# ZenGo-X/multi-party-ecdsa

Hardware: AMD Instinct MI355X
Metric: GG20 signatures/sec (t=1, n=3; all parties of each session on the node's GPUs) + Paillier-2048 modexp/s per GPU (higher is better)
Workload: dtype u32 limbs (radix 2^29) / u64 accumulators

## Files before the change

multi_party_ecdsa_amd/csrc/mpe_internal.h:

```cpp
#pragma once
#include <hip/hip_runtime.h>
#include <stdint.h>
#include <new>
#include <utility>
#include <string>
#include <vector>

#include "../../include/mpecdsa_hip.h"
#include "mpe_kernels_heavy.h"
#include "mpe_sched.h"

struct mpe_ctx {
  int device = 0;
  int cus = 256;
  int fb_window_bits = 13;
  int window_bits = 0;
  bool ec_lane_groups = true;
  bool adaptive_lanes = true;
  bool use_pown = true;
  bool use_pair = true;
  bool use_multiexp = true;
  bool use_crt = true;
  bool use_fixed_base = true;
  bool use_sliding = true;
  int wide_div = 4;
  int device_share = 1;
  int xwide_div = 16;
  bool merge_xn = true;
  int use_prio = 1;
  int ladder_prio = 1;
  int use_crt_n = 1;
  int no_pdl_ahead = 0;
  int no_r1_dlog_first = 0;
  int no_r1_inversion_ahead = 0;
  int merge_r1_quarters = 1;
  bool merge_r1 = true;
  size_t fb_budget_bytes = 0;
  int modexp_waves_per_cu = 8;
  int fb_split = 0;
  int gg20_trace = 0;
  int sampler_max_attempts = 128;
  int no_primaries = 0;
  int no_elect = 0;
  int grid_mode = 2;
  void* tables[6] = {nullptr, nullptr, nullptr, nullptr, nullptr, nullptr};
  size_t tables_bytes[6] = {0, 0, 0, 0, 0, 0};
  hipStream_t aux[3] = {nullptr, nullptr, nullptr};
  hipEvent_t ev_fork[2] = {nullptr, nullptr}, ev_join[3] = {nullptr, nullptr, nullptr};
  hipEvent_t ev_ahead = nullptr;
  hipEvent_t ev_mid = nullptr;
  bool aux_ready = false;
  bool allow_par = true;
  int par_items = 32768;
  void* ws = nullptr;
  size_t ws_bytes = 0, ws_off = 0;
  int ws_hold = 0;
  size_t ws_top = 0;
  void* sess_buf = nullptr;
  size_t sess_bytes = 0;
  bool sess_in_use = false;
  void* slab_buf = nullptr;
  size_t slab_bytes = 0;
  mpe_launch_info last = {};
  mpe_encoding enc = {};
  bool prof_on = false;
  struct ProfEvt { hipEvent_t a, b; int kind, bits, exp_words, batch, exp2_words; int wave_trips; };
  std::vector<ProfEvt> prof;
  uint32_t* prof_ctr = nullptr;
  int prof_ctr_cap = 0;
};

struct mpe_modset {
// ... 98 lines not shown
```

multi_party_ecdsa_amd/csrc/mpe_lib.hip:

```cpp
#include <string.h>
#include <initializer_list>
#include <mutex>
#include "mpe_internal.h"
#include "mpe_ec.h"

using namespace mpe;

thread_local std::string g_last_error;
void mpe_set_error(const char* what, hipError_t e) { g_last_error = std::string(what) + ": " + hipGetErrorString(e); }
void mpe_set_error_msg(const char* what) { g_last_error = what; }

namespace mpe {

int ws_reserve(mpe_ctx* ctx, size_t bytes, hipStream_t st) {
  if (ctx->ws_hold) {
    if (ctx->ws_off + bytes + ctx->ws_top > ctx->ws_bytes) { mpe_set_error_msg("workspace: the shared reservation is too small"); return MPE_E_NOMEM; }
    return MPE_OK;
  }
  ctx->ws_off = 0;
  if (bytes + ctx->ws_top <= ctx->ws_bytes) return MPE_OK;
  if (ctx->ws_top) { mpe_set_error_msg("workspace: cannot grow while a caller keeps arrays at its top"); return MPE_E_NOMEM; }
  if (ctx->ws) { (void)hipStreamSynchronize(st); (void)hipFree(ctx->ws); ctx->ws = nullptr; ctx->ws_bytes = 0; }
  const size_t want = bytes + (bytes >> 2) + (1u << 20);
  hipError_t e = hipMalloc(&ctx->ws, want);
// ... 235 lines not shown
extern "C" {

const char* mpe_version(void) { return "mpecdsa-hip 0.6.0 (gfx950)"; }
const char* mpe_last_error(void) { return g_last_error.c_str(); }

void mpe_encoding_default(mpe_encoding* e) {
  if (!e) return;
  memset(e, 0, sizeof *e);
  e->ck_salt = 0x4B5A656Eu;
  for (int i = 0; i < 4; ++i) e->ord_dlog[i] = e->ord_cdlog[i] = (uint8_t)i;
  for (int i = 0; i < 8; ++i) e->ord_pedersen[i] = e->ord_heg[i] = e->ord_ecddh[i] = (uint8_t)i;
}
static bool is_perm(const uint8_t* o, int n) {
  unsigned seen = 0;
  for (int i = 0; i < n; ++i) { if (o[i] >= n || (seen >> o[i]) & 1u) return false; seen |= 1u << o[i]; }
  return true;
}
int mpe_ctx_set_encoding(mpe_ctx* ctx, const mpe_encoding* e) {
  if (!ctx || !e) return MPE_E_ARG;
  if (e->chain_point > 1 || e->zero_bytes > 1 || e->ck_mask_order > 1 || e->reserved != 0 || !is_perm(e->ord_dlog, 3) ||
      !is_perm(e->ord_pedersen, 5) || !is_perm(e->ord_heg, 7) || !is_perm(e->ord_ecddh, 6) || !is_perm(e->ord_cdlog, 4)) {
    mpe_set_error_msg("mpe_ctx_set_encoding: a flag is not 0/1 or an order is not a permutation");
    return MPE_E_ARG;
  }
  ctx->enc = *e;
  return MPE_OK;
}
int mpe_ctx_set_device_share(mpe_ctx* ctx, int contexts) {
  if (!ctx || contexts < 1 || contexts > 64) return MPE_E_ARG;
  ctx->device_share = contexts;
  return MPE_OK;
}
int mpe_ctx_get_encoding(const mpe_ctx* ctx, mpe_encoding* out) {
  if (!ctx || !out) return MPE_E_ARG;
  *out = ctx->enc;
  return MPE_OK;
}

namespace mpe {
struct CtxOption {
  const char* key;
  long lo, hi;
  void (*set)(mpe_ctx*, long);
  long (*get)(const mpe_ctx*);
};
#define MPE_OPT_BOOL_OFF(name, field) {name, 0, 1, [](mpe_ctx* c, long v) { c->field = !v; }, [](const mpe_ctx* c) -> long { return c->field ? 0 : 1; }}
#define MPE_OPT_INT(name, lo, hi, field) {name, lo, hi, [](mpe_ctx* c, long v) { c->field = (decltype(c->field))v; }, [](const mpe_ctx* c) -> long { return (long)c->field; }}
static const CtxOption kCtxOptions[] = {
    MPE_OPT_BOOL_OFF("no_fixed_base", use_fixed_base),
    MPE_OPT_BOOL_OFF("no_crt", use_crt),
    MPE_OPT_BOOL_OFF("no_multiexp", use_multiexp),
    MPE_OPT_BOOL_OFF("no_pair", use_pair),
    MPE_OPT_BOOL_OFF("no_pown", use_pown),
    MPE_OPT_BOOL_OFF("no_sliding", use_sliding),
    MPE_OPT_BOOL_OFF("no_par", allow_par),
    MPE_OPT_BOOL_OFF("no_wide", adaptive_lanes),
    MPE_OPT_BOOL_OFF("no_ec_lane_groups", ec_lane_groups),
    MPE_OPT_BOOL_OFF("no_merge_xn", merge_xn),
    MPE_OPT_BOOL_OFF("no_merge_r1", merge_r1),
    MPE_OPT_INT("fb_window_bits", 4, 16, fb_window_bits),
    MPE_OPT_INT("window_bits", 0, 6, window_bits),
    MPE_OPT_INT("wide_div", 1, 64, wide_div),
    MPE_OPT_INT("merge_r1_quarters", 0, 64, merge_r1_quarters),
    MPE_OPT_INT("no_r1_inversion_ahead", 0, 1, no_r1_inversion_ahead),
    MPE_OPT_BOOL_OFF("no_prio", use_prio),
    MPE_OPT_INT("no_pdl_ahead", 0, 1, no_pdl_ahead),
    MPE_OPT_BOOL_OFF("no_crt_n", use_crt_n),
    MPE_OPT_INT("no_r1_dlog_first", 0, 1, no_r1_dlog_first),
    MPE_OPT_INT("xwide_div", 0, 1 << 20, xwide_div),
    MPE_OPT_INT("waves_per_cu", 1, 8, modexp_waves_per_cu),
    MPE_OPT_INT("grid_mode", 0, 2, grid_mode),
    MPE_OPT_INT("fb_split", 0, 64, fb_split),
    MPE_OPT_INT("gg20_trace", 0, 1, gg20_trace),
    MPE_OPT_INT("sampler_max_attempts", 1, 1 << 20, sampler_max_attempts),
    MPE_OPT_INT("no_primaries", 0, 1, no_primaries),
    MPE_OPT_INT("no_elect", 0, 1, no_elect),
    {"fb_budget_mb", 0, 1 << 20, [](mpe_ctx* c, long v) { c->fb_budget_bytes = (size_t)v << 20; }, [](const mpe_ctx* c) -> long { return (long)(c->fb_budget_bytes >> 20); }},
};
#undef MPE_OPT_BOOL_OFF
#undef MPE_OPT_INT
extern "C++" void ctx_copy_options(mpe_ctx* dst, const mpe_ctx* src) {
  for (const CtxOption& o : kCtxOptions) o.set(dst, o.get(src));
}
}

int mpe_ctx_set_option(mpe_ctx* ctx, const char* key, const char* value) {
  if (!ctx || !key || !value) return MPE_E_ARG;
  if (!strcmp(key, "grid")) {
    const int m = !strcmp(value, "equal") ? 0 : (!strcmp(value, "full") ? 1 : (!strcmp(value, "hybrid") ? 2 : -1));
    if (m < 0) { mpe_set_error_msg("mpe_ctx_set_option: grid = equal | full | hybrid"); return MPE_E_ARG; }
    ctx->grid_mode = m;
    return MPE_OK;
  }
  if (!strcmp(key, "no_adaptive_lanes")) {
    const bool off = atoi(value) != 0;
    ctx->adaptive_lanes = !off; ctx->ec_lane_groups = !off;
    return MPE_OK;
  }
  for (const mpe::CtxOption& o : mpe::kCtxOptions) {
    if (strcmp(key, o.key)) continue;
    char* end = nullptr;
    const long v = strtol(value, &end, 10);
    if (end == value || *end || v < o.lo || v > o.hi) {
      mpe_set_error_msg((std::string("mpe_ctx_set_option: ") + key + " takes an integer in [" + std::to_string(o.lo) + ", " + std::to_string(o.hi) + "]").c_str());
      return MPE_E_ARG;
    }
// ... 205 lines not shown
```

multi_party_ecdsa_amd/csrc/mpe_pairexp.h:

```cpp
#pragma once
#include <type_traits>
#include "mpe_internal.h"
#include "mpe_small.h"

namespace mpe {

template <class C>
struct PairLds {
  static constexpr int B0 = 0;
  static constexpr int B1 = C::K;
  static constexpr int M = 2 * C::K;
  static constexpr int KC = 3 * C::K;
  static constexpr int pick_stride() {
    constexpr int per_half = (C::GROUPS >= 2) ? C::GROUPS / 2 : 1;
    for (int s = 4 * C::K + 2;; s += 2) {
      bool ok = true;
      for (int a = 0; a < per_half && ok; ++a)
        for (int b = a + 1; b < per_half; ++b)
          if (((a * s) & 31) == ((b * s) & 31)) { ok = false; break; }
      if (ok) return s;
    }
  }
  static constexpr int STRIDE = pick_stride();
  static constexpr int WORDS = STRIDE * C::GROUPS;
// ... 66 lines not shown
      const uint32_t bj = bp[r];
      c[r] += (uint64_t)a[0] * bj;
      const uint32_t m = bcast0_masked<C::TPI>((uint32_t)c[r] * n0inv, maskv);
      if (STORE_M) mp[r] = m;
#pragma unroll
      for (int i = 1; i < L; ++i) c[(r + i) % L] += (uint64_t)a[i] * bj;
#pragma unroll
      for (int i = 0; i < L; ++i) c[(r + i) % L] += (uint64_t)m * n[i];
      c[(r + 1) % L] += c[r] >> W;
      c[r] = (uint64_t)(pull_next((uint32_t)c[r]) & maskv);
    };
    static_for<0, C::STEPS % L>(step);
    if (jj == C::STEPS / L) break;
    static_for<C::STEPS % L, L>(step);
  }
  cios_finish<C>(res, c, ln);
}

template <class C>
__device__ __forceinline__ void cios2(uint32_t (&res)[C::L], uint64_t (&c)[C::L], const uint32_t (&a0)[C::L],
                                      const uint32_t (&a1)[C::L], const uint32_t* __restrict__ bl0,
                                      const uint32_t* __restrict__ bl1, const uint32_t (&n)[C::L], uint32_t n0inv,
                                      const Lane& ln) {
  constexpr int L = C::L, W = C::W;
  uint32_t maskv = C::MASK;
  asm volatile("" : "+v"(maskv));
#pragma unroll 1
  for (int jj = 0;; ++jj) {
    const uint32_t* bp0 = bl0 + jj * L;
    const uint32_t* bp1 = bl1 + jj * L;
    auto step = [&](auto rc) {
      constexpr int r = decltype(rc)::value;
      const uint32_t b0j = bp0[r], b1j = bp1[r];
      c[r] += (uint64_t)a0[0] * b1j;
      c[r] += (uint64_t)a1[0] * b0j;
      const uint32_t m = bcast0_masked<C::TPI>((uint32_t)c[r] * n0inv, maskv);
#pragma unroll
      for (int i = 1; i < L; ++i) {
        c[(r + i) % L] += (uint64_t)a0[i] * b1j;
        c[(r + i) % L] += (uint64_t)a1[i] * b0j;
      }
#pragma unroll
      for (int i = 0; i < L; ++i) c[(r + i) % L] += (uint64_t)m * n[i];
      c[(r + 1) % L] += c[r] >> W;
      c[r] = (uint64_t)(pull_next((uint32_t)c[r]) & maskv);
    };
    static_for<0, C::STEPS % L>(step);
    if (jj == C::STEPS / L) break;
    static_for<C::STEPS % L, L>(step);
  }
  cios_finish<C>(res, c, ln);
}

template <class C>
__device__ __forceinline__ void pairmul(uint32_t (&r0)[C::L], uint32_t (&r1)[C::L], const uint32_t (&a0)[C::L],
                                        const uint32_t (&a1)[C::L], uint32_t* gl, const uint32_t (&n)[C::L],
                                        uint32_t n0inv, bool sq, bool half, const Lane& ln) {
  using PL = PairLds<C>;
  constexpr int L = C::L;
  uint64_t c[L];
#pragma unroll
  for (int i = 0; i < L; ++i) c[i] = 0;
  cios1<C, true>(r0, c, a0, gl + PL::B0, gl + PL::M, n, n0inv, ln);
  wave_lds_sync();
  if (half) {
#pragma unroll
    for (int i = 0; i < L; ++i) r1[i] = 0;
    return;
  }
#pragma unroll
  for (int i = 0; i < L; ++i) {
    uint32_t mi = gl[PL::M + ln.t * L + i];
    if (C::STEPS == C::K - 1) {
      if (i == L - 1) mi = (ln.t == C::TPI - 1) ? 0u : mi;
    } else if (C::STEPS < C::K) {
      mi = (ln.t * L + i < C::STEPS) ? mi : 0u;
    }
    c[i] = (uint64_t)(gl[PL::KC + ln.t * L + i] - mi);
  }
  wave_lds_sync();
#pragma unroll
  for (int i = 0; i < L; ++i) gl[PL::M + ln.t * L + i] = r0[i];
  if (sq) {
    cios1<C, false>(r1, c, a1, gl + PL::B1, gl + PL::M, n, n0inv, ln);
  } else {
    cios2<C>(r1, c, a0, a1, gl + PL::B0, gl + PL::B1, n, n0inv, ln);
  }
  wave_lds_sync();
#pragma unroll
  for (int i = 0; i < L; ++i) r0[i] = gl[PL::M + ln.t * L + i];
}

template <class C>
__device__ __forceinline__ void copy_pair_to_lds(uint32_t* gl, const uint32_t* __restrict__ src, const Lane& ln, int off1 = C::K) {
  using PL = PairLds<C>;
#pragma unroll
  for (int i = 0; i < C::L; ++i) {
    gl[PL::B0 + ln.t + C::TPI * i] = src[ln.t + C::TPI * i];
    gl[PL::B1 + ln.t + C::TPI * i] = src[off1 + ln.t + C::TPI * i];
  }
}
template <class C>
__device__ __forceinline__ void copy_row_to_lds(uint32_t* gl, const uint32_t* __restrict__ row, const Lane& ln) {
  using PL = PairLds<C>;
  static_assert(PL::B0 == 0 && PL::B1 == C::K && (2 * C::K) % 4 == 0 && PL::STRIDE % 2 == 0, "B0 | B1 must be one 8-byte aligned run");
  constexpr int CHUNKS = 2 * C::K / 4;
  const uint4* __restrict__ r4 = reinterpret_cast<const uint4*>(row);
  uint2* l2 = reinterpret_cast<uint2*>(gl + PL::B0);
#pragma unroll
  for (int i = 0; i < (CHUNKS + C::TPI - 1) / C::TPI; ++i) {
    const int ch = ln.t + C::TPI * i;
    if ((i + 1) * C::TPI <= CHUNKS || ch < CHUNKS) {
      const uint4 v = r4[ch];
      l2[2 * ch] = make_uint2(v.x, v.y);
      l2[2 * ch + 1] = make_uint2(v.z, v.w);
    }
  }
}

template <class C>
__global__ void __launch_bounds__(64) pairset_setup_kernel(int count, const uint32_t* __restrict__ moduli,
                                                           uint32_t* __restrict__ n_limbs, uint32_t* __restrict__ n0inv_out,
                                                           uint32_t* __restrict__ one, uint32_t* __restrict__ r2,
                                                           uint32_t* __restrict__ tp, uint32_t* __restrict__ kc) {
  __shared__ uint32_t lds[C::LDS_WORDS];
  constexpr int KS = pair_kstore(C::BITS);
  const Lane ln = make_lane<C>();
  uint32_t* gl = lds + ln.g * C::STRIDE;
  const int slot = blockIdx.x * C::GROUPS + ln.g;
  const bool active = slot < count;
  const int idx = active ? slot : count - 1;
  stage_words<C>(gl, moduli + (size_t)idx * C::K32, ln);
  wave_lds_sync();
  uint32_t n[C::L];
  limbs_from_words<C>(n, gl, ln);
  const uint32_t w0 = gl[0];
  uint32_t inv = w0;
#pragma unroll
  for (int i = 0; i < 5; ++i) inv *= 2u - w0 * inv;
  const uint32_t n0inv = (0u - inv) & C::MASK;
  wave_lds_sync();

  int64_t x0[C::L], x1[C::L];
#pragma unroll
  for (int i = 0; i < C::L; ++i) { x0[i] = (ln.t == 0 && i == 0) ? 1 : 0; x1[i] = 0; }
  auto store_pair = [&](uint32_t* dst) {
    if (!active) return;
#pragma unroll
    for (int i = 0; i < C::L; ++i) {
      dst[(size_t)idx * 2 * KS + ln.t * C::L + i] = (uint32_t)x0[i];
      dst[(size_t)idx * 2 * KS + KS + ln.t * C::L + i] = (uint32_t)x1[i];
    }
  };
  constexpr int WK = C::W * C::STEPS;
#pragma unroll 1
  for (int d = 1; d <= 2 * WK; ++d) {
#pragma unroll
    for (int i = 0; i < C::L; ++i) x0[i] *= 2;
    full_normalize<C>(x0, ln);
    const bool cy = cmp_ge<C>(x0, n, ln);
    if (cy) {
#pragma unroll
      for (int i = 0; i < C::L; ++i) x0[i] -= (int64_t)n[i];
      full_normalize<C>(x0, ln);
    }
#pragma unroll
    for (int i = 0; i < C::L; ++i) x1[i] *= 2;
    if (cy && ln.t == 0) x1[0] += 1;
    full_normalize<C>(x1, ln);
    if (cmp_ge<C>(x1, n, ln)) {
#pragma unroll
// ... 59 lines not shown
  __syncthreads();
  for (int k = threadIdx.x; k < nkeys; k += blockDim.x)
    if (sh[k]) atomicAdd(&cnt[k], sh[k]);
}
static __global__ void __launch_bounds__(64) key_scan_kernel(int nkeys, const int32_t* __restrict__ cnt, int32_t* __restrict__ cursor) {
  __shared__ int32_t part[64];
  const int per = (nkeys + 63) / 64, lo = threadIdx.x * per, hi = lo + per < nkeys ? lo + per : nkeys;
  int32_t s = 0;
  for (int k = lo; k < hi; ++k) s += cnt[k];
  part[threadIdx.x] = s;
  __syncthreads();
  int32_t base = 0;
  for (int t = 0; t < (int)threadIdx.x; ++t) base += part[t];
  for (int k = lo; k < hi; ++k) { cursor[k] = base; base += cnt[k]; }
}
static __global__ void __launch_bounds__(256) key_scatter_kernel(int batch, Rows sel, int nkeys, int32_t* __restrict__ cursor, int32_t* __restrict__ perm) {
  extern __shared__ int32_t sh[];
  for (int k = threadIdx.x; k < 2 * nkeys; k += blockDim.x) sh[k] = 0;
  __syncthreads();
  const int i = blockIdx.x * blockDim.x + threadIdx.x;
  const int mi = i < batch ? sel_index(sel, i) : -1;
  const int local = mi >= 0 ? atomicAdd(&sh[mi], 1) : 0;
  __syncthreads();
  for (int k = threadIdx.x; k < nkeys; k += blockDim.x)
    if (sh[k]) sh[nkeys + k] = atomicAdd(&cursor[k], sh[k]);
  __syncthreads();
  if (mi >= 0) perm[sh[nkeys + mi] + local] = i;
}

static __global__ void pair_slide_audit_kernel(int batch, int groups, Rows exps, int exp_words, int wb, int exp2_words,
                                               const int32_t* __restrict__ perm, uint32_t* __restrict__ ctr) {
  const int u = blockIdx.x * blockDim.x + threadIdx.x;
  if (u * groups >= batch) return;
  const uint32_t* first = nullptr;
  bool same = true;
  for (int g = 0; g < groups; ++g) {
    const int inst = u * groups + g;
    const int pos = inst < batch ? inst : batch - 1;
    const uint32_t* ex = row_of(exps, perm ? perm[pos] : pos);
    if (g == 0) first = ex; else same = same && ex == first;
  }
  if (!same) return;
  uint32_t val = 0;
  const int lo = slide_window((UniformWords)(uintptr_t)first, exp_words, exp_words * 32 - 1, wb, val);
  if (lo < 0 || (exp2_words && lo < 32 * exp2_words)) return;
  atomicAdd(ctr, 1u);
}

#ifdef MPE_WAVE_TRACE
static __device__ unsigned long long* g_wave_trace;
static __device__ unsigned g_wave_trace_cap, g_wave_trace_n;
#endif

template <class C, bool SLIDE>
__global__ void __launch_bounds__(64) __attribute__((amdgpu_waves_per_eu(2, 2))) pair_modexp_kernel(int batch, PairsetView ps, Rows mod_sel, Rows base, Rows exps,
                                                         int exp_words, int wb, Rows base2, Rows exps2, int exp2_words,
                                                         int half, uint32_t* __restrict__ out, uint32_t* __restrict__ tables,
                                                         const int32_t* __restrict__ perm, int slide, SchedArgs sched) {
  using PL = PairLds<C>;
  __shared__ __attribute__((aligned(16))) uint32_t lds[PL::WORDS];
  const Lane ln = make_lane<C>();
  uint32_t* gl = lds + ln.g * PL::STRIDE;
  constexpr int K2 = 2 * C::K;
  const int slot = blockIdx.x * C::GROUPS + ln.g;
  const int nslots = gridDim.x * C::GROUPS;
  const bool dual = base2.p != nullptr;
  const int TE = 1 << wb;
  uint32_t* tab = tables + (size_t)slot * (TE + (dual ? 16 : 0)) * K2;
  uint32_t* tab2 = tab + (size_t)TE * K2;
  const int nwin = (exp_words * 32 + wb - 1) / wb;
  const int nwin2 = dual ? exp2_words * 8 : 0;
  const int top_bit = (nwin - 1) * wb;
  const int words1 = base.words ? base.words : 2 * C::K32, words2 = base2.words ? base2.words : 2 * C::K32;
  WaveSched ws;
  ws.init(sched);

#pragma unroll 1
  for (;;) {
    int ubase;
    if (!ws.next(sched, batch, nslots, C::GROUPS, ubase)) break;
#ifdef MPE_WAVE_TRACE
    const int trip = ws.trip - 1;
    const unsigned long long wt_m0 = __builtin_amdgcn_s_memtime(), wt_r0 = __builtin_amdgcn_s_memrealtime();
#endif
    const int inst = ubase + ln.g;
    const bool active = inst < batch;
    const int pos = active ? inst : batch - 1;
    const int idx = (SLIDE && perm) ? perm[pos] : pos;
    const int mi = sel_index(mod_sel, idx);
    const uint32_t* ex = row_of(exps, idx);
    const uint32_t* ex2 = dual ? row_of(exps2, idx) : ex;
    bool sl_rt = false;
    int sw_lo = -1;
    uint32_t sw_val = 0;
    UniformWords exu = nullptr;
    if (SLIDE && slide) {
      const uint64_t ea = (uint64_t)(uintptr_t)ex;
      const uint32_t e_lo = __builtin_amdgcn_readfirstlane((uint32_t)ea), e_hi = __builtin_amdgcn_readfirstlane((uint32_t)(ea >> 32));
      sl_rt = __ballot(ea != (((uint64_t)e_hi << 32) | e_lo)) == 0;
      exu = (UniformWords)(((uint64_t)e_hi << 32) | e_lo);
      if (sl_rt) {
        sw_lo = slide_window(exu, exp_words, exp_words * 32 - 1, wb, sw_val);
        if (sw_lo < 0 || (dual && sw_lo < 32 * exp2_words)) sl_rt = false;
      }
    }

    uint32_t n[C::L];
    constexpr int KS = pair_kstore(C::BITS);
    load_owner<C>(n, ps.n_limbs + (size_t)mi * KS, ln);
    const uint32_t n0inv = ps.n0inv[mi];
    {
      const uint32_t* kc = ps.kc + (size_t)mi * KS;
#pragma unroll
      for (int i = 0; i < C::L; ++i)
        gl[PL::KC + ln.t + C::TPI * i] = kc[ln.t + C::TPI * i] + ((ln.t + C::TPI * i) < C::STEPS ? C::MASK : 0u);
      uint32_t t0[C::L], t1[C::L];
      load_owner<C>(t0, ps.one + (size_t)mi * 2 * KS, ln);
      load_owner<C>(t1, ps.one + (size_t)mi * 2 * KS + KS, ln);
      store_owner<C>(tab, t0, ln);
      store_owner<C>(tab + C::K, t1, ln);
    }

    const bool sl = SLIDE && sl_rt;
    uint32_t cur0[C::L], cur1[C::L];
    int which = 0;
    const uint32_t* bw = row_of(base, idx);
    int kin = (words1 + C::K32 - 1) / C::K32 - 1;
    load_words_as_limbs<C>(cur0, gl, bw + kin * C::K32, words1 - kin * C::K32, ln);
#pragma unroll
    for (int i = 0; i < C::L; ++i) cur1[i] = 0;
    int ph = kin > 0 ? PP_IN : PP_MONT;
    --kin;
    int k = 0, b = top_bit;
#pragma unroll 1
    while (ph != PP_DONE) {
      bool sq = false;
      if (ph == PP_IN) {
        copy_pair_to_lds<C>(gl, ps.tp + (size_t)mi * 2 * KS, ln, KS);
      } else if (ph == PP_MONT) {
        copy_pair_to_lds<C>(gl, ps.r2 + (size_t)mi * 2 * KS, ln, KS);
      } else if (ph == PP_TAB) {
        if (k == 1 && !(sl && !which)) { put_limbs<C>(gl + PL::B0, cur0, ln); put_limbs<C>(gl + PL::B1, cur1, ln); }
      } else if (ph == PP_SQ || (SLIDE && ph == PP_TSQ)) {
        put_limbs<C>(gl + PL::B0, cur0, ln);
#pragma unroll
        for (int i = 0; i < C::L; ++i) gl[PL::B1 + ln.t * C::L + i] = cur0[i] << 1;
        sq = true;
      } else if (ph == PP_MUL1) {
        const uint32_t w = sl ? sw_val : exp_window(ex, exp_words, b / wb, wb);
#ifndef MPE_NARROW_COPY
        copy_row_to_lds<C>(gl, tab + (size_t)w * K2, ln);
#else
        copy_pair_to_lds<C>(gl, tab + (size_t)w * K2, ln);
#endif
      } else if (ph == PP_MUL2) {
        const int wi = b >> 2;
        const uint32_t w = (ex2[wi >> 3] >> ((wi & 7) * 4)) & 15u;
#ifndef MPE_NARROW_COPY
        copy_row_to_lds<C>(gl, w ? tab2 + (size_t)w * K2 : tab, ln);
#else
        copy_pair_to_lds<C>(gl, w ? tab2 + (size_t)w * K2 : tab, ln);
#endif
      } else {
#pragma unroll
        for (int i = 0; i < C::L; ++i) {
          gl[PL::B0 + ln.t * C::L + i] = (ln.t == 0 && i == 0) ? 1u : 0u;
          gl[PL::B1 + ln.t * C::L + i] = 0u;
        }
      }
      wave_lds_sync();
      uint32_t r0[C::L], r1[C::L];
      pairmul<C>(r0, r1, cur0, cur1, gl, n, n0inv, sq, half != 0, ln);
      wave_lds_sync();
#pragma unroll
      for (int i = 0; i < C::L; ++i) { cur0[i] = r0[i]; cur1[i] = r1[i]; }

      bool tables_done = false;
      if (ph == PP_IN) {
        uint32_t ch[C::L];
        load_words_as_limbs<C>(ch, gl, bw + kin * C::K32, C::K32, ln);
        int64_t z[C::L];
#pragma unroll
        for (int i = 0; i < C::L; ++i) z[i] = (int64_t)cur0[i] + (int64_t)ch[i];
        full_normalize<C>(z, ln);
#pragma unroll
        for (int i = 0; i < C::L; ++i) cur0[i] = (uint32_t)z[i];
        if (--kin < 0) ph = PP_MONT;
      } else if (ph == PP_MONT) {
        uint32_t* T = which ? tab2 : tab;
        store_owner<C>(T + K2, cur0, ln);
        store_owner<C>(T + K2 + C::K, cur1, ln);
        k = 1;
        ph = (sl && !which) ? PP_TSQ : PP_TAB;
      } else if (SLIDE && ph == PP_TSQ) {
        put_limbs<C>(gl + PL::B0, cur0, ln);
        put_limbs<C>(gl + PL::B1, cur1, ln);
        __builtin_amdgcn_fence(__ATOMIC_SEQ_CST, "workgroup");
        load_owner<C>(cur0, tab + K2, ln);
        load_owner<C>(cur1, tab + K2 + C::K, ln);
        ph = PP_TAB;
      } else if (ph == PP_TAB) {
        uint32_t* T = which ? tab2 : tab;
        const int step = (sl && !which) ? 2 : 1;
        k += step;
        store_owner<C>(T + (size_t)k * K2, cur0, ln);
        store_owner<C>(T + (size_t)k * K2 + C::K, cur1, ln);
        if (k > (which ? 14 : TE - 2)) {
          if (!which && dual) {
            which = 1;
            bw = row_of(base2, idx);
            kin = (words2 + C::K32 - 1) / C::K32 - 1;
            load_words_as_limbs<C>(cur0, gl, bw + kin * C::K32, words2 - kin * C::K32, ln);
#pragma unroll
            for (int i = 0; i < C::L; ++i) cur1[i] = 0;
            ph = kin > 0 ? PP_IN : PP_MONT;
            --kin;
          } else {
            tables_done = true;
          }
        }
      } else if (ph == PP_FINAL) {
        ph = PP_DONE;
      } else {
        if (ph == PP_SQ) --b;
        if (ph == PP_MUL1 && sl) sw_lo = slide_window(exu, exp_words, b - 1, wb, sw_val);
        const bool m1 = ph == PP_SQ && (sl ? b == sw_lo : (b % wb) == 0);
        const bool m2 = ph != PP_MUL2 && dual && (b & 3) == 0 && (b >> 2) < nwin2;
        ph = m1 ? PP_MUL1 : (m2 ? PP_MUL2 : (b == 0 ? PP_FINAL : PP_SQ));
      }
      if (tables_done) {
        __builtin_amdgcn_fence(__ATOMIC_SEQ_CST, "workgroup");
        const uint32_t w = sl ? sw_val : exp_window(ex, exp_words, nwin - 1, wb);
        load_owner<C>(cur0, tab + (size_t)w * K2, ln);
        load_owner<C>(cur1, tab + (size_t)w * K2 + C::K, ln);
        b = sl ? sw_lo : top_bit;
        if (sl) sw_lo = slide_window(exu, exp_words, b - 1, wb, sw_val);
        ph = b == 0 ? PP_FINAL : PP_SQ;
      }
    }
    {
      int64_t z[C::L];
#pragma unroll
      for (int i = 0; i < C::L; ++i) z[i] = (int64_t)cur0[i];
      full_normalize<C>(z, ln);
      const bool ge = cmp_ge<C>(z, n, ln);
      if (ge) {
#pragma unroll
        for (int i = 0; i < C::L; ++i) z[i] -= (int64_t)n[i];
        full_normalize<C>(z, ln);
      }
#pragma unroll
      for (int i = 0; i < C::L; ++i) { cur0[i] = (uint32_t)z[i]; z[i] = (int64_t)cur1[i]; }
      if (ge && !half && ln.t == 0) z[0] += 1;
      full_normalize<C>(z, ln);
#pragma unroll 1
      for (int pass = 0; pass < 2; ++pass) {
        if (cmp_ge<C>(z, n, ln)) {
#pragma unroll
          for (int i = 0; i < C::L; ++i) z[i] -= (int64_t)n[i];
          full_normalize<C>(z, ln);
        }
      }
#pragma unroll
      for (int i = 0; i < C::L; ++i) cur1[i] = (uint32_t)z[i];
    }
    store_limbs_as_words<C>(out + (size_t)idx * 2 * C::K32, gl, cur0, active, ln);
    store_limbs_as_words<C>(out + (size_t)idx * 2 * C::K32 + C::K32, gl, cur1, active, ln);
#ifdef MPE_WAVE_TRACE
    if (g_wave_trace && threadIdx.x == 0) {
      const unsigned long long wt_m1 = __builtin_amdgcn_s_memtime(), wt_r1 = __builtin_amdgcn_s_memrealtime();
      const unsigned at = atomicAdd(&g_wave_trace_n, 1u);
      if (at < g_wave_trace_cap) {
        unsigned long long* w = g_wave_trace + (size_t)at * 8;
        w[0] = ((unsigned long long)gridDim.x << 32) | blockIdx.x;
        w[1] = ((unsigned long long)(unsigned)batch << 32) | ((unsigned)trip << 16) | ((unsigned)C::L << 8) | ((unsigned)(ws.role != 0) << 2) | ((unsigned)(half != 0) << 1) | (unsigned)(SLIDE ? 1 : 0);
        w[2] = ((unsigned long long)__builtin_amdgcn_s_getreg((31 << 11) | 20) << 32) | __builtin_amdgcn_s_getreg((31 << 11) | 4);
        w[3] = wt_m0; w[4] = wt_m1; w[5] = wt_r0; w[6] = wt_r1;
        w[7] = ((unsigned long long)(unsigned)C::BITS << 32) | (unsigned)exp_words;
      }
    }
#endif
  }
}

template <int H>
__global__ void pair_finish_kernel(int B, Rows mod_sel, const uint32_t* __restrict__ mod_words, uint32_t* __restrict__ out) {
  MPE_FOREGROUND();
  const int i = blockIdx.x * blockDim.x + threadIdx.x;
  if (i >= B) return;
  uint32_t z0[H], z1[H], nn[H], r[2 * H];
  sm::copy(z0, out + (size_t)i * 2 * H, H);
  sm::copy(z1, out + (size_t)i * 2 * H + H, H);
  sm::copy(nn, mod_words + (size_t)sel_index(mod_sel, i) * H, H);
  sm::mul(r, z1, H, nn, H);
  sm::add(r, 2 * H, r, 2 * H, z0, H);
  sm::copy(out + (size_t)i * 2 * H, r, 2 * H);
}

}

namespace mpe {

#ifdef MPE_WAVE_TRACE
static int wave_trace_arm_impl(void* buf, unsigned cap) {
  const unsigned zero = 0;
  if (hipMemcpyToSymbol(HIP_SYMBOL(g_wave_trace), &buf, sizeof buf) != hipSuccess) return MPE_E_HIP;
  if (hipMemcpyToSymbol(HIP_SYMBOL(g_wave_trace_cap), &cap, sizeof cap) != hipSuccess) return MPE_E_HIP;
  if (hipMemcpyToSymbol(HIP_SYMBOL(g_wave_trace_n), &zero, sizeof zero) != hipSuccess) return MPE_E_HIP;
  return MPE_OK;
}
static int wave_trace_count_impl(unsigned* n) {
  return hipMemcpyFromSymbol(n, HIP_SYMBOL(g_wave_trace_n), sizeof *n) == hipSuccess ? MPE_OK : MPE_E_HIP;
}
#endif

template <class C>
int pairset_create_impl(int count, const uint32_t* d_moduli, mpe_pairset** out, hipStream_t st) {
  mpe_pairset* ps = new (std::nothrow) mpe_pairset();
  if (!ps) return MPE_E_NOMEM;
  ps->half_bits = C::BITS;
  ps->count = count;
  ps->mod_words = d_moduli;
  const size_t K = pair_kstore(C::BITS), words = (size_t)count * (K + 1 + 3 * 2 * K + K);
  static_assert(pair_kstore(C::BITS) >= C::K, "the stored constants must hold the layout's limbs");
  hipError_t e = hipMalloc(&ps->blob, words * 4);
  if (e != hipSuccess) { delete ps; mpe_set_error("hipMalloc(pairset)", e); return MPE_E_NOMEM; }
  (void)hipMemsetAsync(ps->blob, 0, words * 4, st);
  uint32_t* p = (uint32_t*)ps->blob;
  ps->n_limbs = p; p += count * K;
  ps->n0inv = p; p += count;
  ps->one = p; p += count * 2 * K;
  ps->r2 = p; p += count * 2 * K;
  ps->tp = p; p += count * 2 * K;
  ps->kc = p;
  hipLaunchKernelGGL(pairset_setup_kernel<C>, dim3((count + C::GROUPS - 1) / C::GROUPS), dim3(64), 0, st, count, d_moduli,
                     ps->n_limbs, ps->n0inv, ps->one, ps->r2, ps->tp, ps->kc);
  e = hipGetLastError();
  if (e != hipSuccess) { (void)hipFree(ps->blob); delete ps; mpe_set_error("pairset_setup_kernel", e); return MPE_E_HIP; }
  *out = ps;
  return MPE_OK;
}

template <class C>
int pair_modexp_impl(mpe_ctx* ctx, const mpe_pairset* ps, int batch, Rows mod_sel, Rows base, Rows exps, int exp_words,
                     Rows base2, Rows exps2, int exp2_words, int half, uint32_t* d_out, hipStream_t st, int public_exp) {
  const int units = (batch + C::GROUPS - 1) / C::GROUPS;
  const int grid = ladder_grid(ctx, units, ctx->cus * ctx->modexp_waves_per_cu);
  int wb = exp_words <= 8 ? 4 : (exp_words < 48 ? 5 : 6);
  if (ctx->window_bits) wb = ctx->window_bits;
  const bool dual = base2.p != nullptr;
  if (dual && (exp2_words <= 0 || 32 * exp2_words > ((exp_words * 32 + wb - 1) / wb - 1) * wb)) {
    mpe_set_error_msg("pair modexp: the second exponent must be shorter than the first");
    return MPE_E_ARG;
  }
  const size_t need = (size_t)grid * C::GROUPS * (((size_t)1 << wb) + (dual ? 16 : 0)) * 2 * C::K * sizeof(uint32_t);
  const int slide = (public_exp && ctx->use_sliding && !half && exp_words >= 16 && wb >= 5) ? 1 : 0;
  const bool by_key = slide && ps->count > 1 && (mod_sel.idx || mod_sel.stride) && ps->count <= 4096 && batch > C::GROUPS;
  const size_t extra = (by_key ? ((size_t)batch + 2 * (size_t)ps->count + 64) * sizeof(int32_t) : 0) + SCHED_WORDS * sizeof(int32_t);
  uint32_t* tabs = tables_for(ctx, need + extra, st);
  if (!tabs) return MPE_E_NOMEM;
  SchedArgs sched = ladder_sched(ctx, units, ctx->cus * ctx->modexp_waves_per_cu, (int32_t*)((char*)tabs + need + extra) - SCHED_WORDS, st);
  if (sched.prio == 1) sched.prio = 2;
  const int32_t* perm = nullptr;
  if (by_key) {
    int32_t* pm = (int32_t*)((char*)tabs + need);
    int32_t *cnt = pm + batch, *cursor = cnt + ps->count;
    (void)hipMemsetAsync(cnt, 0, (size_t)ps->count * sizeof(int32_t), st);
    const int nb = (batch + 255) / 256;
    hipLaunchKernelGGL(key_hist_kernel, dim3(nb), dim3(256), (size_t)ps->count * 4, st, batch, mod_sel, ps->count, cnt);
    hipLaunchKernelGGL(key_scan_kernel, dim3(1), dim3(64), 0, st, ps->count, cnt, cursor);
    hipLaunchKernelGGL(key_scatter_kernel, dim3(nb), dim3(256), (size_t)ps->count * 8, st, batch, mod_sel, ps->count, cursor, pm);
    perm = pm;
  }
  PairsetView v{ps->n_limbs, ps->n0inv, ps->one, ps->r2, ps->tp, ps->kc, ps->count};
  prof_begin(ctx, st, half ? 4 : (slide ? 6 : 3), half ? C::BITS : 2 * C::BITS, exp_words, batch, dual ? exp2_words : 0);
  if (slide)
    hipLaunchKernelGGL((pair_modexp_kernel<C, true>), dim3(grid), dim3(64), 0, st, batch, v, mod_sel, base, exps, exp_words, wb, base2,
                       exps2, exp2_words, half, d_out, tabs, perm, slide, sched);
  else
    hipLaunchKernelGGL((pair_modexp_kernel<C, false>), dim3(grid), dim3(64), 0, st, batch, v, mod_sel, base, exps, exp_words, wb, base2,
                       exps2, exp2_words, half, d_out, tabs, perm, slide, sched);
  prof_end(ctx, st);
  if (slide) {
    if (uint32_t* ctr = prof_counter(ctx, units))
      hipLaunchKernelGGL(pair_slide_audit_kernel, dim3(blocks_for(units, 64)), dim3(64), 0, st, batch, (int)C::GROUPS, exps,
                         exp_words, wb, dual ? exp2_words : 0, perm, ctr);
  }
  hipLaunchKernelGGL(pair_finish_kernel<C::K32>, dim3(blocks_for(batch, 64)), dim3(64), 0, st, batch, mod_sel, ps->mod_words, d_out);
  hipError_t e = hipGetLastError();
  if (e != hipSuccess) { mpe_set_error("pair_modexp_kernel", e); return MPE_E_HIP; }
  ctx->last.waves = grid;
  ctx->last.ints_per_wave = C::GROUPS;
  ctx->last.limbs = 2 * C::K;
  ctx->last.limb_bits = C::W;
  ctx->last.lds_bytes_per_wave = PairLds<C>::WORDS * 4;
  ctx->last.table_scratch_bytes = need;
  return MPE_OK;
}

}
```

multi_party_ecdsa_amd/engine.py:

```python
import ctypes as C
import os

import numpy as np
import torch

from . import _native as N
N_ = N
from .words import ints_to_words, words_to_ints


def _dev_u32(arr_np, device):
    return torch.from_numpy(arr_np.view(np.int32)).to(device)


def _to_np_u32(t):
    return t.detach().cpu().numpy().view(np.uint32)


_ENV_OPTIONS = ["no_fixed_base", "no_crt", "no_multiexp", "no_pair", "no_pown", "no_sliding", "no_par", "no_wide", "no_adaptive_lanes",
                "no_merge_xn", "no_merge_r1", "fb_window_bits", "window_bits", "wide_div", "xwide_div", "waves_per_cu", "grid", "fb_budget_mb",
                "fb_split", "gg20_trace", "sampler_max_attempts", "no_elect", "no_primaries", "merge_r1_quarters",
                "no_r1_inversion_ahead", "no_r1_dlog_first", "no_prio", "no_pdl_ahead", "no_crt_n"]


def options_from_env(env=None):
    env = os.environ if env is None else env
    out = {}
    for k in _ENV_OPTIONS:
        v = env.get("MPE_" + k.upper())
        if v is not None and v != "":
            out[k] = v
    if env.get("MPE_GRID_EQUAL"):
        out["grid"] = "equal"
    return out


class Context:
    def __init__(self, device=0, encoding=None, options=None):
        if not torch.cuda.is_available():
            raise N.MpeError("no GPU visible: the HIP path cannot run (there is no CPU fallback)")
        self.device = torch.device("cuda", device)
        h = C.c_void_p()
        N.check(N.lib.mpe_ctx_create(C.byref(h), device), "mpe_ctx_create")
        self.h = h
        if encoding is not None:
            self.set_encoding(encoding)
        self.options = {}
        for k, v in {**options_from_env(), **(options or {})}.items():
            self.set_option(k, v)

    def set_option(self, key, value):
        N.check(N.lib.mpe_ctx_set_option(self.h, str(key).encode(), str(int(value) if isinstance(value, bool) else value).encode()), f"mpe_ctx_set_option({key})")
        self.options[key] = value

    def get_option(self, key):
        v = C.c_long(0)
        N.check(N.lib.mpe_ctx_get_option(self.h, str(key).encode(), C.byref(v)), f"mpe_ctx_get_option({key})")
        return v.value

    def set_device_share(self, contexts):
        N.check(N.lib.mpe_ctx_set_device_share(self.h, int(contexts)), "mpe_ctx_set_device_share")

    def set_encoding(self, encoding):
        e = encoding if isinstance(encoding, N.Encoding) else N.Encoding.from_dict(dict(encoding))
        N.check(N.lib.mpe_ctx_set_encoding(self.h, C.byref(e)), "mpe_ctx_set_encoding")

    def encoding(self):
        e = N.Encoding()
        N.check(N.lib.mpe_ctx_get_encoding(self.h, C.byref(e)), "mpe_ctx_get_encoding")
        return e.as_dict()

    def stream(self):
        return C.c_void_p(torch.cuda.current_stream(self.device).cuda_stream)

    def sync(self):
# ... 926 lines not shown
```

Before: 19450.

## Add lean half-width pair modexp variant and register row prefetch for 1024-bit pairs

Adds a compile-time HALF variant of the 1024-bit pair modexp kernel. When only one half is needed, it skips the second CIOS lane, the second table column and the final pair_finish kernel, which halves table storage and multiply work. It also adds a register prefetch of the next window's table row, issued one window ahead so the global load overlaps the squarings. The cost is more template instantiations and extra register pressure from the prefetch buffer, which could lower occupancy.

```diff
diff --git a/multi_party_ecdsa_amd/csrc/mpe_internal.h b/multi_party_ecdsa_amd/csrc/mpe_internal.h
--- a/multi_party_ecdsa_amd/csrc/mpe_internal.h
+++ b/multi_party_ecdsa_amd/csrc/mpe_internal.h
@@ -18,6 +18,8 @@
   bool ec_lane_groups = true;
   bool adaptive_lanes = true;
   bool use_pown = true;
+  bool lean_half = true;
+  bool row_prefetch = true;
   bool use_pair = true;
   bool use_multiexp = true;
   bool use_crt = true;
diff --git a/multi_party_ecdsa_amd/csrc/mpe_lib.hip b/multi_party_ecdsa_amd/csrc/mpe_lib.hip
--- a/multi_party_ecdsa_amd/csrc/mpe_lib.hip
+++ b/multi_party_ecdsa_amd/csrc/mpe_lib.hip
@@ -311,6 +311,8 @@
     MPE_OPT_BOOL_OFF("no_multiexp", use_multiexp),
     MPE_OPT_BOOL_OFF("no_pair", use_pair),
     MPE_OPT_BOOL_OFF("no_pown", use_pown),
+    MPE_OPT_BOOL_OFF("no_lean_half", lean_half),
+    MPE_OPT_BOOL_OFF("no_row_prefetch", row_prefetch),
     MPE_OPT_BOOL_OFF("no_sliding", use_sliding),
     MPE_OPT_BOOL_OFF("no_par", allow_par),
     MPE_OPT_BOOL_OFF("no_wide", adaptive_lanes),
diff --git a/multi_party_ecdsa_amd/csrc/mpe_pairexp.h b/multi_party_ecdsa_amd/csrc/mpe_pairexp.h
--- a/multi_party_ecdsa_amd/csrc/mpe_pairexp.h
+++ b/multi_party_ecdsa_amd/csrc/mpe_pairexp.h
@@ -142,7 +142,7 @@
   cios_finish<C>(res, c, ln);
 }
 
-template <class C>
+template <class C, bool HALF = false>
 __device__ __forceinline__ void pairmul(uint32_t (&r0)[C::L], uint32_t (&r1)[C::L], const uint32_t (&a0)[C::L],
                                         const uint32_t (&a1)[C::L], uint32_t* gl, const uint32_t (&n)[C::L],
                                         uint32_t n0inv, bool sq, bool half, const Lane& ln) {
@@ -151,6 +151,13 @@
   uint64_t c[L];
 #pragma unroll
   for (int i = 0; i < L; ++i) c[i] = 0;
+  if constexpr (HALF) {
+    cios1<C, false>(r0, c, a0, gl + PL::B0, gl + PL::M, n, n0inv, ln);
+    wave_lds_sync();
+#pragma unroll
+    for (int i = 0; i < L; ++i) r1[i] = 0;
+    return;
+  }
   cios1<C, true>(r0, c, a0, gl + PL::B0, gl + PL::M, n, n0inv, ln);
   wave_lds_sync();
   if (half) {
@@ -181,20 +188,20 @@
   for (int i = 0; i < L; ++i) r0[i] = gl[PL::M + ln.t * L + i];
 }
 
-template <class C>
+template <class C, bool HALF = false>
 __device__ __forceinline__ void copy_pair_to_lds(uint32_t* gl, const uint32_t* __restrict__ src, const Lane& ln, int off1 = C::K) {
   using PL = PairLds<C>;
 #pragma unroll
   for (int i = 0; i < C::L; ++i) {
     gl[PL::B0 + ln.t + C::TPI * i] = src[ln.t + C::TPI * i];
-    gl[PL::B1 + ln.t + C::TPI * i] = src[off1 + ln.t + C::TPI * i];
-  }
-}
-template <class C>
+    if (!HALF) gl[PL::B1 + ln.t + C::TPI * i] = src[off1 + ln.t + C::TPI * i];
+  }
+}
+template <class C, int WORDS = 2 * C::K>
 __device__ __forceinline__ void copy_row_to_lds(uint32_t* gl, const uint32_t* __restrict__ row, const Lane& ln) {
   using PL = PairLds<C>;
-  static_assert(PL::B0 == 0 && PL::B1 == C::K && (2 * C::K) % 4 == 0 && PL::STRIDE % 2 == 0, "B0 | B1 must be one 8-byte aligned run");
-  constexpr int CHUNKS = 2 * C::K / 4;
+  static_assert(PL::B0 == 0 && PL::B1 == C::K && WORDS % 4 == 0 && PL::STRIDE % 2 == 0, "B0 | B1 must be one 8-byte aligned run");
+  constexpr int CHUNKS = WORDS / 4;
   const uint4* __restrict__ r4 = reinterpret_cast<const uint4*>(row);
   uint2* l2 = reinterpret_cast<uint2*>(gl + PL::B0);
 #pragma unroll
@@ -207,6 +214,32 @@
     }
   }
 }
+template <class C, int WORDS>
+struct RowPrefetch {
+  static constexpr int CHUNKS = WORDS / 4, PER = (CHUNKS + C::TPI - 1) / C::TPI;
+  uint4 v[PER];
+  __device__ __forceinline__ void load(const uint32_t* __restrict__ row, const Lane& ln) {
+    const uint4* __restrict__ r4 = reinterpret_cast<const uint4*>(row);
+#pragma unroll
+    for (int i = 0; i < PER; ++i) {
+      const int ch = ln.t + C::TPI * i;
+      if ((i + 1) * C::TPI <= CHUNKS || ch < CHUNKS) v[i] = r4[ch];
+    }
+  }
+  __device__ __forceinline__ void put(uint32_t* gl, const Lane& ln) const {
+    using PL = PairLds<C>;
+    static_assert(PL::B0 == 0 && WORDS % 4 == 0 && WORDS <= 2 * C::K && PL::STRIDE % 2 == 0, "rows land in B0 | B1, 8-byte aligned");
+    uint2* l2 = reinterpret_cast<uint2*>(gl + PL::B0);
+#pragma unroll
+    for (int i = 0; i < PER; ++i) {
+      const int ch = ln.t + C::TPI * i;
+      if ((i + 1) * C::TPI <= CHUNKS || ch < CHUNKS) {
+        l2[2 * ch] = make_uint2(v[i].x, v[i].y);
+        l2[2 * ch + 1] = make_uint2(v[i].z, v[i].w);
+      }
+    }
+  }
+};
 
 template <class C>
 __global__ void __launch_bounds__(64) pairset_setup_kernel(int count, const uint32_t* __restrict__ moduli,
@@ -372,16 +405,25 @@
 static __device__ unsigned g_wave_trace_cap, g_wave_trace_n;
 #endif
 
+template <class Base, bool H, bool P>
+struct PairVariant : Base {};
+template <class C>
+struct PairVariantOf { static constexpr bool HALF = false, PF = false; };
+template <class Base, bool H, bool P>
+struct PairVariantOf<PairVariant<Base, H, P>> { static constexpr bool HALF = H, PF = P; };
+
 template <class C, bool SLIDE>
 __global__ void __launch_bounds__(64) __attribute__((amdgpu_waves_per_eu(2, 2))) pair_modexp_kernel(int batch, PairsetView ps, Rows mod_sel, Rows base, Rows exps,
                                                          int exp_words, int wb, Rows base2, Rows exps2, int exp2_words,
                                                          int half, uint32_t* __restrict__ out, uint32_t* __restrict__ tables,
                                                          const int32_t* __restrict__ perm, int slide, SchedArgs sched) {
   using PL = PairLds<C>;
+  constexpr bool HALF = PairVariantOf<C>::HALF, PF = PairVariantOf<C>::PF;
+  static_assert(!(SLIDE && (HALF || PF)), "the lean and prefetching variants run the fixed windows only");
   __shared__ __attribute__((aligned(16))) uint32_t lds[PL::WORDS];
   const Lane ln = make_lane<C>();
   uint32_t* gl = lds + ln.g * PL::STRIDE;
-  constexpr int K2 = 2 * C::K;
+  constexpr int K2 = HALF ? C::K : 2 * C::K;
   const int slot = blockIdx.x * C::GROUPS + ln.g;
   const int nslots = gridDim.x * C::GROUPS;
   const bool dual = base2.p != nullptr;
@@ -430,16 +472,19 @@
     load_owner<C>(n, ps.n_limbs + (size_t)mi * KS, ln);
     const uint32_t n0inv = ps.n0inv[mi];
     {
-      const uint32_t* kc = ps.kc + (size_t)mi * KS;
-#pragma unroll
-      for (int i = 0; i < C::L; ++i)
-        gl[PL::KC + ln.t + C::TPI * i] = kc[ln.t + C::TPI * i] + ((ln.t + C::TPI * i) < C::STEPS ? C::MASK : 0u);
+      if constexpr (!HALF) {
+        const uint32_t* kc = ps.kc + (size_t)mi * KS;
+#pragma unroll
+        for (int i = 0; i < C::L; ++i)
+          gl[PL::KC + ln.t + C::TPI * i] = kc[ln.t + C::TPI * i] + ((ln.t + C::TPI * i) < C::STEPS ? C::MASK : 0u);
+      }
       uint32_t t0[C::L], t1[C::L];
       load_owner<C>(t0, ps.one + (size_t)mi * 2 * KS, ln);
-      load_owner<C>(t1, ps.one + (size_t)mi * 2 * KS + KS, ln);
+      if (!HALF) load_owner<C>(t1, ps.one + (size_t)mi * 2 * KS + KS, ln);
       store_owner<C>(tab, t0, ln);
-      store_owner<C>(tab + C::K, t1, ln);
-    }
+      if (!HALF) store_owner<C>(tab + C::K, t1, ln);
+    }
+    RowPrefetch<C, K2> pf;
 
     const bool sl = SLIDE && sl_rt;
     uint32_t cur0[C::L], cur1[C::L];
@@ -456,41 +501,49 @@
     while (ph != PP_DONE) {
       bool sq = false;
       if (ph == PP_IN) {
-        copy_pair_to_lds<C>(gl, ps.tp + (size_t)mi * 2 * KS, ln, KS);
+        copy_pair_to_lds<C, HALF>(gl, ps.tp + (size_t)mi * 2 * KS, ln, KS);
       } else if (ph == PP_MONT) {
-        copy_pair_to_lds<C>(gl, ps.r2 + (size_t)mi * 2 * KS, ln, KS);
+        copy_pair_to_lds<C, HALF>(gl, ps.r2 + (size_t)mi * 2 * KS, ln, KS);
       } else if (ph == PP_TAB) {
-        if (k == 1 && !(sl && !which)) { put_limbs<C>(gl + PL::B0, cur0, ln); put_limbs<C>(gl + PL::B1, cur1, ln); }
+        if (k == 1 && !(sl && !which)) { put_limbs<C>(gl + PL::B0, cur0, ln); if (!HALF) put_limbs<C>(gl + PL::B1, cur1, ln); }
       } else if (ph == PP_SQ || (SLIDE && ph == PP_TSQ)) {
         put_limbs<C>(gl + PL::B0, cur0, ln);
-#pragma unroll
-        for (int i = 0; i < C::L; ++i) gl[PL::B1 + ln.t * C::L + i] = cur0[i] << 1;
+        if constexpr (!HALF) {
+#pragma unroll
+          for (int i = 0; i < C::L; ++i) gl[PL::B1 + ln.t * C::L + i] = cur0[i] << 1;
+        }
         sq = true;
       } else if (ph == PP_MUL1) {
-        const uint32_t w = sl ? sw_val : exp_window(ex, exp_words, b / wb, wb);
+        if constexpr (PF) {
+          pf.put(gl, ln);
+          const int wn = b / wb - 1;
+          pf.load(tab + (size_t)(wn >= 0 ? exp_window(ex, exp_words, wn, wb) : 0u) * K2, ln);
+        } else {
+          const uint32_t w = sl ? sw_val : exp_window(ex, exp_words, b / wb, wb);
 #ifndef MPE_NARROW_COPY
-        copy_row_to_lds<C>(gl, tab + (size_t)w * K2, ln);
+          copy_row_to_lds<C, K2>(gl, tab + (size_t)w * K2, ln);
 #else
-        copy_pair_to_lds<C>(gl, tab + (size_t)w * K2, ln);
+          copy_pair_to_lds<C, HALF>(gl, tab + (size_t)w * K2, ln);
 #endif
+        }
       } else if (ph == PP_MUL2) {
         const int wi = b >> 2;
         const uint32_t w = (ex2[wi >> 3] >> ((wi & 7) * 4)) & 15u;
 #ifndef MPE_NARROW_COPY
-        copy_row_to_lds<C>(gl, w ? tab2 + (size_t)w * K2 : tab, ln);
+        copy_row_to_lds<C, K2>(gl, w ? tab2 + (size_t)w * K2 : tab, ln);
 #else
-        copy_pair_to_lds<C>(gl, w ? tab2 + (size_t)w * K2 : tab, ln);
+        copy_pair_to_lds<C, HALF>(gl, w ? tab2 + (size_t)w * K2 : tab, ln);
 #endif
       } else {
 #pragma unroll
         for (int i = 0; i < C::L; ++i) {
           gl[PL::B0 + ln.t * C::L + i] = (ln.t == 0 && i == 0) ? 1u : 0u;
-          gl[PL::B1 + ln.t * C::L + i] = 0u;
+          if (!HALF) gl[PL::B1 + ln.t * C::L + i] = 0u;
         }
       }
       wave_lds_sync();
       uint32_t r0[C::L], r1[C::L];
-      pairmul<C>(r0, r1, cur0, cur1, gl, n, n0inv, sq, half != 0, ln);
+      pairmul<C, HALF>(r0, r1, cur0, cur1, gl, n, n0inv, sq, half != 0, ln);
       wave_lds_sync();
 #pragma unroll
       for (int i = 0; i < C::L; ++i) { cur0[i] = r0[i]; cur1[i] = r1[i]; }
@@ -509,7 +562,7 @@
       } else if (ph == PP_MONT) {
         uint32_t* T = which ? tab2 : tab;
         store_owner<C>(T + K2, cur0, ln);
-        store_owner<C>(T + K2 + C::K, cur1, ln);
+        if (!HALF) store_owner<C>(T + K2 + C::K, cur1, ln);
         k = 1;
         ph = (sl && !which) ? PP_TSQ : PP_TAB;
       } else if (SLIDE && ph == PP_TSQ) {
@@ -524,7 +577,7 @@
         const int step = (sl && !which) ? 2 : 1;
         k += step;
         store_owner<C>(T + (size_t)k * K2, cur0, ln);
-        store_owner<C>(T + (size_t)k * K2 + C::K, cur1, ln);
+        if (!HALF) store_owner<C>(T + (size_t)k * K2 + C::K, cur1, ln);
         if (k > (which ? 14 : TE - 2)) {
           if (!which && dual) {
             which = 1;
@@ -552,12 +605,19 @@
         __builtin_amdgcn_fence(__ATOMIC_SEQ_CST, "workgroup");
         const uint32_t w = sl ? sw_val : exp_window(ex, exp_words, nwin - 1, wb);
         load_owner<C>(cur0, tab + (size_t)w * K2, ln);
-        load_owner<C>(cur1, tab + (size_t)w * K2 + C::K, ln);
+        if (!HALF) load_owner<C>(cur1, tab + (size_t)w * K2 + C::K, ln);
+        if constexpr (PF) pf.load(tab + (size_t)(nwin >= 2 ? exp_window(ex, exp_words, nwin - 2, wb) : 0u) * K2, ln);
         b = sl ? sw_lo : top_bit;
         if (sl) sw_lo = slide_window(exu, exp_words, b - 1, wb, sw_val);
         ph = b == 0 ? PP_FINAL : PP_SQ;
       }
     }
+    if constexpr (HALF) {
+      reduce_once<C>(cur0, n, ln);
+      store_limbs_as_words<C>(out + (size_t)idx * 2 * C::K32, gl, cur0, active, ln);
+      if (active)
+        for (int q = ln.t; q < C::K32; q += C::TPI) out[(size_t)idx * 2 * C::K32 + C::K32 + q] = 0u;
+    } else {
     {
       int64_t z[C::L];
 #pragma unroll
@@ -586,6 +646,7 @@
     }
     store_limbs_as_words<C>(out + (size_t)idx * 2 * C::K32, gl, cur0, active, ln);
     store_limbs_as_words<C>(out + (size_t)idx * 2 * C::K32 + C::K32, gl, cur1, active, ln);
+    }
 #ifdef MPE_WAVE_TRACE
     if (g_wave_trace && threadIdx.x == 0) {
       const unsigned long long wt_m1 = __builtin_amdgcn_s_memtime(), wt_r1 = __builtin_amdgcn_s_memrealtime();
@@ -669,11 +730,14 @@
   int wb = exp_words <= 8 ? 4 : (exp_words < 48 ? 5 : 6);
   if (ctx->window_bits) wb = ctx->window_bits;
   const bool dual = base2.p != nullptr;
+  constexpr bool PAIR_PF = C::BITS == 1024 && C::L <= 9;
+  const bool lean = C::BITS == 1024 && half && ctx->lean_half;
+  const bool pf = C::BITS == 1024 && ctx->row_prefetch && (lean || PAIR_PF);
   if (dual && (exp2_words <= 0 || 32 * exp2_words > ((exp_words * 32 + wb - 1) / wb - 1) * wb)) {
     mpe_set_error_msg("pair modexp: the second exponent must be shorter than the first");
     return MPE_E_ARG;
   }
-  const size_t need = (size_t)grid * C::GROUPS * (((size_t)1 << wb) + (dual ? 16 : 0)) * 2 * C::K * sizeof(uint32_t);
+  const size_t need = (size_t)grid * C::GROUPS * (((size_t)1 << wb) + (dual ? 16 : 0)) * (lean ? 1 : 2) * C::K * sizeof(uint32_t);
   const int slide = (public_exp && ctx->use_sliding && !half && exp_words >= 16 && wb >= 5) ? 1 : 0;
   const bool by_key = slide && ps->count > 1 && (mod_sel.idx || mod_sel.stride) && ps->count <= 4096 && batch > C::GROUPS;
   const size_t extra = (by_key ? ((size_t)batch + 2 * (size_t)ps->count + 64) * sizeof(int32_t) : 0) + SCHED_WORDS * sizeof(int32_t);
@@ -694,19 +758,36 @@
   }
   PairsetView v{ps->n_limbs, ps->n0inv, ps->one, ps->r2, ps->tp, ps->kc, ps->count};
   prof_begin(ctx, st, half ? 4 : (slide ? 6 : 3), half ? C::BITS : 2 * C::BITS, exp_words, batch, dual ? exp2_words : 0);
-  if (slide)
-    hipLaunchKernelGGL((pair_modexp_kernel<C, true>), dim3(grid), dim3(64), 0, st, batch, v, mod_sel, base, exps, exp_words, wb, base2,
-                       exps2, exp2_words, half, d_out, tabs, perm, slide, sched);
-  else
-    hipLaunchKernelGGL((pair_modexp_kernel<C, false>), dim3(grid), dim3(64), 0, st, batch, v, mod_sel, base, exps, exp_words, wb, base2,
-                       exps2, exp2_words, half, d_out, tabs, perm, slide, sched);
+#define MPE_PAIR_LAUNCH(LAYOUT, SL)                                                                                             \
+  hipLaunchKernelGGL((pair_modexp_kernel<LAYOUT, SL>), dim3(grid), dim3(64), 0, st, batch, v, mod_sel, base, exps, exp_words, wb, base2, \
+                     exps2, exp2_words, half, d_out, tabs, perm, slide, sched)
+  bool done = false;
+  if constexpr (C::BITS == 1024) {
+    if (!slide && (lean || pf)) {
+      using LeanPf = PairVariant<C, true, true>;
+      using Lean = PairVariant<C, true, false>;
+      using Pf = PairVariant<C, false, true>;
+      if (lean && pf) MPE_PAIR_LAUNCH(LeanPf, false);
+      else if (lean) MPE_PAIR_LAUNCH(Lean, false);
+      else if constexpr (PAIR_PF) MPE_PAIR_LAUNCH(Pf, false);
+      done = true;
+    }
+  }
+  if (done) {
+  } else if (slide) {
+    MPE_PAIR_LAUNCH(C, true);
+  } else {
+    MPE_PAIR_LAUNCH(C, false);
+  }
+#undef MPE_PAIR_LAUNCH
   prof_end(ctx, st);
   if (slide) {
     if (uint32_t* ctr = prof_counter(ctx, units))
       hipLaunchKernelGGL(pair_slide_audit_kernel, dim3(blocks_for(units, 64)), dim3(64), 0, st, batch, (int)C::GROUPS, exps,
                          exp_words, wb, dual ? exp2_words : 0, perm, ctr);
   }
-  hipLaunchKernelGGL(pair_finish_kernel<C::K32>, dim3(blocks_for(batch, 64)), dim3(64), 0, st, batch, mod_sel, ps->mod_words, d_out);
+  if (!lean)
+    hipLaunchKernelGGL(pair_finish_kernel<C::K32>, dim3(blocks_for(batch, 64)), dim3(64), 0, st, batch, mod_sel, ps->mod_words, d_out);
   hipError_t e = hipGetLastError();
   if (e != hipSuccess) { mpe_set_error("pair_modexp_kernel", e); return MPE_E_HIP; }
   ctx->last.waves = grid;
diff --git a/multi_party_ecdsa_amd/engine.py b/multi_party_ecdsa_amd/engine.py
--- a/multi_party_ecdsa_amd/engine.py
+++ b/multi_party_ecdsa_amd/engine.py
@@ -20,7 +20,7 @@
 _ENV_OPTIONS = ["no_fixed_base", "no_crt", "no_multiexp", "no_pair", "no_pown", "no_sliding", "no_par", "no_wide", "no_adaptive_lanes",
                 "no_merge_xn", "no_merge_r1", "fb_window_bits", "window_bits", "wide_div", "xwide_div", "waves_per_cu", "grid", "fb_budget_mb",
                 "fb_split", "gg20_trace", "sampler_max_attempts", "no_elect", "no_primaries", "merge_r1_quarters",
-                "no_r1_inversion_ahead", "no_r1_dlog_first", "no_prio", "no_pdl_ahead", "no_crt_n"]
+                "no_r1_inversion_ahead", "no_r1_dlog_first", "no_prio", "no_pdl_ahead", "no_crt_n", "no_lean_half", "no_row_prefetch"]
 
 
 def options_from_env(env=None):
```

Result: no change. 19600 (median of 6 runs) (+0.8%).
